# MayeulCassier/Matrix-Factorization-With-Comparison-Data

Measured on AMD Instinct MI355X. Metric: triplet-updates/sec, higher is better.
Workload: dtype f32

## Files before the change

matrix-factorization-with-comparison-data_amd/csrc/resident.hip:

```cpp
#include <cstring>
#include <mutex>
#include <utility>
#include <vector>

#include "resident_kernel.h"

#define MFCD_DECL(d)                                                                                                  \
    extern "C" int mfcd_resident_launch_d##d(const mfcd_detail::ResidentArgs *, int, int, void *) __attribute__((weak)); \
    extern "C" int mfcd_resident_occupancy_d##d(int, int, int, int) __attribute__((weak));
MFCD_DECL(2) MFCD_DECL(4) MFCD_DECL(8) MFCD_DECL(16) MFCD_DECL(32) MFCD_DECL(64) MFCD_DECL(128) MFCD_DECL(256)
#undef MFCD_DECL

namespace mfcd_detail {

int g_resident_math = 1;
Tuning g_tune;

typedef int (*ResidentLauncher)(const ResidentArgs *, int, int, void *);
typedef int (*ResidentOccupancy)(int, int, int, int);

static ResidentLauncher launcher_for(int d)
{
    switch (d) {
        case 2: return mfcd_resident_launch_d2;
        case 4: return mfcd_resident_launch_d4;
        case 8: return mfcd_resident_launch_d8;
        case 16: return mfcd_resident_launch_d16;
        case 32: return mfcd_resident_launch_d32;
        case 64: return mfcd_resident_launch_d64;
        case 128: return mfcd_resident_launch_d128;
        case 256: return mfcd_resident_launch_d256;
        default: return nullptr;
    }
}

static ResidentOccupancy occupancy_for(int d)
{
    switch (d) {
        case 2: return mfcd_resident_occupancy_d2;
        case 4: return mfcd_resident_occupancy_d4;
        case 8: return mfcd_resident_occupancy_d8;
        case 16: return mfcd_resident_occupancy_d16;
        case 32: return mfcd_resident_occupancy_d32;
        case 64: return mfcd_resident_occupancy_d64;
        case 128: return mfcd_resident_occupancy_d128;
        case 256: return mfcd_resident_occupancy_d256;
        default: return nullptr;
    }
}

int resident_lookahead(int64_t N, int B, int n, int m)
{
    int la = g_tune.lookahead >= 0 ? g_tune.lookahead : 4;
    if (B > 64) la = 0;
    if (N + 64 * 16 >= ((int64_t)1 << 31)) la = 0;
    if (g_tune.lookahead < 0 && (int64_t)(n + m) < (int64_t)96 * B) la = 0;
    return la > 16 ? 16 : (la < 0 ? 0 : la);
}

static int resident_blocks_per_cu(int d, int Q, int look, int fast, int bf16)
{
    static std::mutex mu;
    static std::vector<std::pair<long long, int>> cache;
    const long long key = ((((long long)d * 64 + Q) * 16 + look) * 2 + fast) * 2 + bf16;
    std::lock_guard<std::mutex> lock(mu);
    for (auto &e : cache)
        if (e.first == key) return e.second;
    int occ = 0;
    if (ResidentOccupancy fn = occupancy_for(d)) occ = fn(Q, look, fast, bf16);
    if (occ > 8) occ = 8;
    if (occ < 0) occ = 0;
    cache.emplace_back(key, occ);
    return occ;
}

static int resident_default_q(int n, int m, int d, int num_cus)
{
    if (d < 2 || d > 256 || (d & (d - 1)) != 0 || num_cus <= 0) return 0;
    const int64_t T = (int64_t)(n + m) * d;
    static const int kQ[5] = {1, 2, 4, 16, 32};
    for (int Q : kQ) {
        if ((64 * Q) % d != 0) continue;
        const int64_t nw = (T + 64 * (int64_t)Q - 1) / (64 * Q);
        if (nw <= (int64_t)num_cus * (Q <= 2 ? 16 : 8) && nw <= kResidentMaxWaves) return Q;
    }
    return 0;
}

ResidentEvents resident_events(int B, int n, int m, int d, int num_cus)
{
    ResidentEvents ev{0, 0, 0};
    const int Q = resident_default_q(n, m, d, num_cus);
    if (!Q || B > 64) return ev;
    ev.rows_per_wave = 64 * Q / d;
    ev.waves = (int)(((int64_t)(n + m) * d + 64 * (int64_t)Q - 1) / (64 * Q));
    const double h = 2.0 * 3.0 * B * ev.rows_per_wave / (double)(n + m);
    for (int ts = 8; ts >= 4; --ts)
        if (h * ((1 << ts) + kResidentEventLook) <= 20.0) {
            ev.tshift = ts;
            break;
        }
    return ev;
}

ResidentPlan plan_resident(int64_t N, int B, int n, int m, int d, int num_cus, bool bf16, int ev_tshift)
{
    ResidentPlan pl{};
    pl.ok = false;
    if (d < 2 || d > 256 || (d & (d - 1)) != 0 || num_cus <= 0 || !launcher_for(d)) return pl;
    const int64_t T = (int64_t)(n + m) * d;
    int look = resident_lookahead(N, B, n, m);
    const bool fast = g_resident_math != 0;
    if (ev_tshift < 0) ev_tshift = resident_events(B, n, m, d, num_cus).tshift;
    if (ev_tshift == 0) look = 0;
    static const int kQ[5] = {1, 2, 4, 16, 32};
    for (int qi = 0; qi < 5; ++qi) {
        const int Q = kQ[qi];
        if ((64 * Q) % d != 0) continue;
        const int64_t nw = (T + 64 * (int64_t)Q - 1) / (64 * Q);
        if (nw <= (int64_t)num_cus * (Q <= 2 ? 16 : 8) && nw <= kResidentMaxWaves) {
            const int occ = resident_blocks_per_cu(d, Q, look, fast, bf16);
            const int blocks = (int)((nw + 3) / 4);
            if (occ > 0 && (int64_t)blocks > (int64_t)occ * num_cus) continue;
            pl.ok = true;
            pl.Q = Q;
            pl.NW = (int)nw;
            pl.blocks = blocks;
            pl.lookahead = look;
            pl.fast_math = fast;
            pl.bf16 = bf16;
            pl.tshift = ev_tshift;
            return pl;
        }
    }
    return pl;
}

constexpr int kInlineStageUnits = 232;
struct InlineStage {
    uint4 v[kInlineStageUnits];
};

size_t train_inline_stage_bytes() { return (size_t)kInlineStageUnits * 16; }

template <bool INLINE>
__global__ __launch_bounds__(256) void train_prologue_kernel(InlineStage inl, const uint4 *__restrict__ stage_host,
                                                             uint4 *__restrict__ stage_dev, int stage_units,
                                                             const mfcd_sample *__restrict__ samples, int64_t N, int B,
                                                             int n, int m, int rows_per_wave, int tshift, int look,
                                                             int64_t nch_cap, mfcd_sample *__restrict__ xs,
                                                             unsigned *__restrict__ ev_cnt, uint4 *__restrict__ ev_ent)
{
    const int64_t t = (int64_t)blockIdx.x * blockDim.x + threadIdx.x;
    if (t < stage_units) {
        if constexpr (INLINE) {
            const uint4 *ka = (const uint4 *)__builtin_amdgcn_kernarg_segment_ptr();
            stage_dev[t] = ka[t];
        } else {
            stage_dev[t] = stage_host[t];
        }
    }
    if (!xs || t >= N) return;
    const RowMap rm = make_row_map(n, m);
    mfcd_sample s = samples[t];
    s.u = rm.vrow_u(s.u);
    s.i = rm.vrow_v(s.i);
    s.j = rm.vrow_v(s.j);
    xs[t] = s;
    if (look <= 0) return;
    const int k = (int)(t / B);
    const unsigned tl = (unsigned)(t - (int64_t)k * B);
    const int w[3] = {s.u / rows_per_wave, s.i / rows_per_wave, s.j / rows_per_wave};
    const unsigned lr[3] = {(unsigned)(s.u - w[0] * rows_per_wave), (unsigned)(s.i - w[1] * rows_per_wave),
                            (unsigned)(s.j - w[2] * rows_per_wave)};
    const int c = k >> tshift;
    const bool copy_back = c > 0 && (k & ((1 << tshift) - 1)) < look;
    uint4 e[3];
    size_t list[3];
    bool need[3];
#pragma unroll
    for (int r = 0; r < 3; ++r) {
        bool first = true;
#pragma unroll
        for (int r2 = 0; r2 < r; ++r2) first = first && w[r2] != w[r];
        need[r] = first;
        unsigned own = 0u, rows = 0u;
#pragma unroll
        for (int r2 = r; r2 < 3; ++r2)
            if (w[r2] == w[r]) {
                own |= 1u << r2;
                rows |= lr[r2] << (10 * r2);
            }
        e[r] = make_uint4(((unsigned)k << 9) | (tl << 3) | own, rows, __float_as_uint(s.z), 0u);
        list[r] = (size_t)w[r] * (size_t)nch_cap + (size_t)c;
    }
    unsigned slot[3] = {0u, 0u, 0u}, slot_back[3] = {0u, 0u, 0u};
#pragma unroll
    for (int r = 0; r < 3; ++r) {
        if (need[r]) slot[r] = atomicAdd(ev_cnt + list[r], 1u);
        if (need[r] && copy_back) slot_back[r] = atomicAdd(ev_cnt + list[r] - 1, 1u);
    }
#pragma unroll
    for (int r = 0; r < 3; ++r) {
        if (need[r] && slot[r] < (unsigned)kEventCap - 1u) ev_ent[list[r] * kEventCap + slot[r]] = e[r];
        if (need[r] && copy_back && slot_back[r] < (unsigned)kEventCap - 1u)
            ev_ent[(list[r] - 1) * kEventCap + slot_back[r]] = e[r];
    }
}

int launch_train_prologue(const void *stage_host, const void *stage_host_devview, void *stage_dev, size_t stage_bytes,
                          const mfcd_sample *samples, int64_t N, int B, int n, int m, int rows_per_wave, int tshift,
                          int look, int64_t nch_cap, mfcd_sample *xs, unsigned *ev_cnt, void *ev_ent, hipStream_t st)
{
    const int units = (int)((stage_bytes + 15) / 16);
    const int64_t items = xs ? (N > units ? N : units) : units;
    constexpr int kPT = 64;
    const dim3 grid((unsigned)((items + kPT - 1) / kPT));
    if (units <= kInlineStageUnits) {
        InlineStage inl;
        std::memcpy(inl.v, stage_host, (size_t)units * 16);
        hipLaunchKernelGGL(train_prologue_kernel<true>, grid, dim3(kPT), 0, st, inl, (const uint4 *)nullptr,
                           (uint4 *)stage_dev, units, samples, N, B, n, m, rows_per_wave, tshift, look, nch_cap, xs,
                           ev_cnt, (uint4 *)ev_ent);
    } else {
        static const InlineStage none{};
        hipLaunchKernelGGL(train_prologue_kernel<false>, grid, dim3(kPT), 0, st, none, (const uint4 *)stage_host_devview,
                           (uint4 *)stage_dev, units, samples, N, B, n, m, rows_per_wave, tshift, look, nch_cap, xs,
                           ev_cnt, (uint4 *)ev_ent);
    }
    MFCD_HIP_TRY(hipGetLastError());
    return 0;
}

int launch_resident_steps(const ResidentPlan &pl, const void *cold_dev, const mfcd_sample *xs, int64_t N, int B, int n,
                          int m, int d, const StepScalars *sc_dev, const AdamStatic &ac, unsigned long long *mailbox,
                          unsigned tag_base, void *loss_terms, unsigned long long *dbg, int K, hipStream_t st)
{
    ResidentArgs a;
    a.dbg = dbg;
    a.cold = (const ResidentCold *)cold_dev;
    a.samples = xs; a.sc = sc_dev; a.mailbox = mailbox; a.loss_terms = loss_terms;
    a.N = N; a.B = B; a.n = n; a.m = m; a.K = K; a.NW = pl.NW; a.ac = ac;
    a.lookahead = pl.lookahead;
    a.tag_base = tag_base;
    a.fast_math = pl.fast_math;
    a.bf16 = pl.bf16;
    ResidentLauncher fn = launcher_for(d);
    if (!fn) return MFCD_EINVAL;
    return fn(&a, pl.Q, pl.blocks, (void *)st);
}

}
```

matrix-factorization-with-comparison-data_amd/csrc/resident_kernel.h:

```cpp
#pragma once
#include "common.h"
#include "train_common.h"

namespace mfcd_detail {

typedef unsigned long long u64;

#define MFCD_LAMBDA_INLINE __attribute__((always_inline))

#ifdef MFCD_RES_STATS
#define RS_NOW() ((u64)__builtin_amdgcn_s_memtime())
#define RS_ADD(slot, val) rs_acc[slot] += (u64)(val)
#else
#define RS_NOW() ((u64)0)
#define RS_ADD(slot, val) ((void)0)
#endif

typedef const __attribute__((address_space(4))) float *ScalarTablePtr;
__device__ __forceinline__ StepScalars load_step_scalars(const StepScalars *table, int k)
{
    const ScalarTablePtr f = (ScalarTablePtr)(table + k);
    StepScalars s;
    s.neg_step_size = f[0];
    s.bc2_sqrt = f[1];
    s.inv_bc2_sqrt = f[2];
    s.pad = 0.0f;
    return s;
}


__device__ __forceinline__ u64 pack_granule(unsigned tag, float v)
{
    return ((u64)tag << 32) | (u64)__float_as_uint(v);
}

__device__ __forceinline__ u64 load_granule(const u64 *p)
{
    return __hip_atomic_load(p, __ATOMIC_RELAXED, __HIP_MEMORY_SCOPE_AGENT);
}

__device__ __forceinline__ void store_granule(u64 *p, unsigned tag, float v)
{
    __hip_atomic_store(p, pack_granule(tag, v), __ATOMIC_RELAXED, __HIP_MEMORY_SCOPE_AGENT);
}

struct RowMap {
    int n, m, c;
    __host__ __device__ int vrow_u(int u) const { return u < c ? 2 * u : 2 * c + (u - c); }
    __host__ __device__ int vrow_v(int i) const { return i < c ? 2 * i + 1 : 2 * c + (i - c); }
    __host__ __device__ int users_below(int x) const
    {
        if (x <= 2 * c) return (x + 1) >> 1;
        return n > c ? c + (x - 2 * c) : c;
    }
    __host__ __device__ int items_below(int x) const
    {
        if (x <= 2 * c) return x >> 1;
        return m > c ? c + (x - 2 * c) : c;
    }
    __host__ __device__ bool is_item(int vr) const { return vr < 2 * c ? (vr & 1) != 0 : m > n; }
    __host__ __device__ int table_row(int vr) const { return vr < 2 * c ? vr >> 1 : c + (vr - 2 * c); }
};
__host__ __device__ inline RowMap make_row_map(int n, int m)
{
    RowMap r;
    r.n = n; r.m = m; r.c = n < m ? n : m;
    return r;
}

constexpr int kEventCap = 64;
constexpr unsigned kEventNone = 0xFFFFFFF8u;
constexpr int kEventMaxLocalRows = 1024;

struct ResidentCold {
    float *U, *V, *mU, *vU, *mV, *vV;
    int *status;
    unsigned long long spin_limit;
    unsigned *ev_cnt;
    uint4 *ev_ent;
    long long nch_cap;
    long long tshift;
    float *loss_out;
    unsigned long long pad[3];
};
static_assert(sizeof(ResidentCold) == 128, "train.hip fills this block as sixteen 8-byte words (kColdBytes)");

struct ResidentArgs {
    const ResidentCold *cold;
    const mfcd_sample *samples;
    const StepScalars *sc;
    u64 *mailbox;
    void *loss_terms;
    u64 *dbg;
    unsigned tag_base;
    int64_t N;
    int B, n, m, K, NW;
    int lookahead;
    int fast_math;
    int bf16;
    AdamStatic ac;
};

__device__ __forceinline__ mfcd_sample load_record(const mfcd_sample *__restrict__ samples, int64_t pos0, int Bk,
                                                   int base, int lane)
{
    mfcd_sample s;
    s.u = s.i = s.j = -0x40000000;
    s.z = 0.0f;
    if (base + lane < Bk) s = samples[pos0 + base + lane];
    return s;
}

struct Masks {
    u64 mu, mi, mj;
};

template <int D, int Q, int LOOK, bool FAST, bool BF16 = false>
__global__ __launch_bounds__(256) __attribute__((amdgpu_waves_per_eu(Q >= 16 ? 2 : 1)))
void resident_train_kernel(ResidentArgs a)
{
    constexpr int S = D >= 64 ? D / 64 : 1;
    constexpr int RPR = D < 64 ? 64 / D : 1;
    constexpr int EW = 64 * Q;
    static_assert(EW % D == 0, "a wave's slice must hold whole rows");
    static_assert(EW / D <= kEventMaxLocalRows, "local row indices are 10-bit fields of an event entry");
    constexpr bool GRL = Q >= 16;
    extern __shared__ __attribute__((aligned(16))) float lds_dyn[];
    const int lane = threadIdx.x & 63;
    const int gw = blockIdx.x * (blockDim.x >> 6) + (threadIdx.x >> 6);
    if (gw >= a.NW) return;

    const int64_t T = (int64_t)(a.n + a.m) * D;
    const int64_t ebase = (int64_t)gw * EW;
    const int Rlo = (int)(ebase / D);
    const int64_t eend = (ebase + EW < T) ? ebase + EW : T;
    const int Rhi = (int)(eend / D);
    const int lcol = lane & (D - 1);
    auto elem_is_item = [&](int64_t e) MFCD_LAMBDA_INLINE { return make_row_map(a.n, a.m).is_item((int)(e / D)); };
    auto elem_offset = [&](int64_t e) MFCD_LAMBDA_INLINE { return (int64_t)make_row_map(a.n, a.m).table_row((int)(e / D)) * D + (e % D); };

#ifdef MFCD_RES_STATS
    u64 rs_acc[8] = {0, 0, 0, 0, 0, 0, 0, 0};
    const u64 rs_t0 = RS_NOW();
    [[maybe_unused]] const u64 rs_abs_t0 = __builtin_amdgcn_s_memrealtime();
    [[maybe_unused]] u64 rs_abs_l0 = 0, rs_abs_l1 = 0;
    [[maybe_unused]] u64 rs_hit[8] = {0, 0, 0, 0, 0, 0, 0, 0};
    [[maybe_unused]] u64 rs_mark = 0;
#endif
    float p[Q], m1[Q], m2[Q], gr[GRL ? 1 : Q];
    float *const lgr = lds_dyn + (threadIdx.x >> 6) * (GRL ? EW : 0);
    auto post = [](float x) MFCD_LAMBDA_INLINE {
        if constexpr (BF16) return (float)(mfcd_bf16)x;
        else return x;
    };
    {
        const ResidentCold c = *a.cold;
#pragma unroll
        for (int q = 0; q < Q; ++q) {
            const int64_t e = ebase + q * 64 + lane;
            p[q] = m1[q] = m2[q] = 0.0f;
            if constexpr (GRL) lgr[q * 64 + lane] = 0.0f;
            if (e < T) {
                const int64_t o = elem_offset(e);
                if (!elem_is_item(e)) { p[q] = BF16 ? (float)((const mfcd_bf16 *)c.U)[o] : c.U[o]; m1[q] = c.mU[o]; m2[q] = c.vU[o]; }
                else { p[q] = BF16 ? (float)((const mfcd_bf16 *)c.V)[o] : c.V[o]; m1[q] = c.mV[o]; m2[q] = c.vV[o]; }
            }
        }
    }

    auto batch_size = [&](int step) MFCD_LAMBDA_INLINE {
        const int64_t pos0 = (int64_t)step * a.B;
        return (int)((a.N - pos0) < a.B ? (a.N - pos0) : a.B);
    };
    auto scan = [&](const mfcd_sample &s, int Bk, int base) MFCD_LAMBDA_INLINE {
        const bool valid = base + lane < Bk;
        const int ru = s.u, ri = s.i, rj = s.j;
        Masks M;
        M.mu = __ballot(valid && ru >= Rlo && ru < Rhi);
        M.mi = __ballot(valid && ri >= Rlo && ri < Rhi);
        M.mj = __ballot(valid && rj >= Rlo && rj < Rhi);
        return M;
    };
    auto reg_of = [&](int lr) MFCD_LAMBDA_INLINE { return D >= 64 ? lr * S : lr / RPR; };

    auto give_up = [&](int step, int64_t pos, int what) MFCD_LAMBDA_INLINE {
        int *const status = a.cold->status;
        if (lane == 0) {
            if (__hip_atomic_exchange(status, 1, __ATOMIC_RELAXED, __HIP_MEMORY_SCOPE_AGENT) == 0 && a.dbg) {
                a.dbg[0] = (u64)gw; a.dbg[1] = (u64)step; a.dbg[2] = (u64)pos; a.dbg[3] = (u64)what;
            }
        }
    };
    auto poll_failed = [&](unsigned &spins, unsigned &limit) MFCD_LAMBDA_INLINE -> bool {
        if (spins == 0) limit = (unsigned)a.cold->spin_limit;
        ++spins;
        if (spins > limit || (spins & 255u) == 0) {
            if (spins > limit ||
                __hip_atomic_load(a.cold->status, __ATOMIC_RELAXED, __HIP_MEMORY_SCOPE_AGENT) != 0)
                return true;
        }
        return false;
    };

    auto store_row = [&](int lr, int64_t slot, unsigned tag) MFCD_LAMBDA_INLINE {
        u64 *dst = a.mailbox + slot * D;
        const int q0 = reg_of(lr);
#pragma unroll
        for (int q = 0; q < Q; ++q) {
            if (q >= q0 && q < q0 + S) {
                if constexpr (D >= 64) {
                    store_granule(dst + (q - q0) * 64 + lane, tag, p[q]);
                } else {
                    if (lane / D == lr % RPR) store_granule(dst + lcol, tag, p[q]);
                }
            }
        }
    };

    auto process_hit = [&](bool own0, bool own1, bool own2, int lr0, int lr1, int lr2, float zz, int64_t pos,
                           unsigned tag, float inv_batch, int step) MFCD_LAMBDA_INLINE -> bool {
        const bool own[3] = {own0, own1, own2};
        const int lrs[3] = {lr0, lr1, lr2};
        const u64 *slot = a.mailbox + pos * 3 * D;

        float row[3][S];
#pragma unroll
        for (int r = 0; r < 3; ++r) {
#pragma unroll
            for (int s2 = 0; s2 < S; ++s2) row[r][s2] = 0.0f;
            if (!own[r]) continue;
            const int q0 = reg_of(lrs[r]);
            if constexpr (D >= 64) {
#pragma unroll
                for (int q = 0; q < Q; ++q)
                    if (q >= q0 && q < q0 + S) row[r][(q * 64 % D) / 64] = p[q];
            } else {
                float sel = 0.0f;
#pragma unroll
                for (int q = 0; q < Q; ++q) sel = (q == q0) ? p[q] : sel;
                const float v = __shfl(sel, (lrs[r] % RPR) * D + lcol, MFCD_WAVE);
                row[r][0] = lane < D ? v : 0.0f;
            }
        }
        unsigned spins = 0, limit = 0;
        [[maybe_unused]] u64 rs_w0 = 0;
        RS_ADD(4, 1ull);
#ifdef MFCD_RES_STAMPS
        { const u64 t = RS_NOW(); rs_hit[0] += t - rs_mark; rs_mark = t; }
#endif
#if defined(MFCD_RES_STAGGER) && MFCD_RES_STAGGER > 0
        {
            u64 ga[3][S], gb[3][S];
            auto issue = [&](u64 (&g)[3][S]) MFCD_LAMBDA_INLINE {
#pragma unroll
                for (int r = 0; r < 3; ++r) {
                    if (own[r]) continue;
#pragma unroll
                    for (int s2 = 0; s2 < S; ++s2) {
                        const int c = lane + 64 * s2;
                        if (c < D) g[r][s2] = load_granule(slot + (int64_t)r * D + c);
                    }
                }
            };
            auto check = [&](const u64 (&g)[3][S]) MFCD_LAMBDA_INLINE -> bool {
                bool ok = true;
#pragma unroll
                for (int r = 0; r < 3; ++r) {
                    if (own[r]) continue;
#pragma unroll
                    for (int s2 = 0; s2 < S; ++s2) {
                        const int c = lane + 64 * s2;
                        if (c < D) {
                            ok = ok && ((unsigned)(g[r][s2] >> 32) == tag);
                            row[r][s2] = __uint_as_float((unsigned)g[r][s2]);
                        }
                    }
                }
                return __all(ok);
            };
            issue(ga);
            if (!check(ga)) {
#ifdef MFCD_RES_STATS
                rs_w0 = RS_NOW();
#endif
                issue(ga);
                __builtin_amdgcn_s_sleep(MFCD_RES_STAGGER);
                issue(gb);
                while (true) {
                    RS_ADD(5, 1);
                    if (poll_failed(spins, limit)) {
                        give_up(step, pos, (own0 ? 1 : 0) | (own1 ? 2 : 0) | (own2 ? 4 : 0));
                        return false;
                    }
                    if (check(ga)) break;
                    issue(ga);
                    if (check(gb)) break;
                    issue(gb);
                }
            }
        }
#else
        while (true) {
            bool ok = true;
#pragma unroll
            for (int r = 0; r < 3; ++r) {
                if (own[r]) continue;
#pragma unroll
                for (int s2 = 0; s2 < S; ++s2) {
                    const int c = lane + 64 * s2;
                    if (c < D) {
                        const u64 gq = load_granule(slot + (int64_t)r * D + c);
                        ok = ok && ((unsigned)(gq >> 32) == tag);
                        row[r][s2] = __uint_as_float((unsigned)gq);
                    }
                }
            }
            if (__all(ok)) break;
#ifdef MFCD_RES_STATS
            if (spins == 0) rs_w0 = RS_NOW();
            RS_ADD(5, 1);
#endif
            if (poll_failed(spins, limit)) {
                give_up(step, pos, (own0 ? 1 : 0) | (own1 ? 2 : 0) | (own2 ? 4 : 0));
                return false;
            }
        }
#endif
#ifdef MFCD_RES_STATS
        if (spins) RS_ADD(2, RS_NOW() - rs_w0);
        else RS_ADD(4, 1ull << 40);
#endif
#ifdef MFCD_RES_STAMPS
        { const u64 t = RS_NOW(); rs_hit[1] += t - rs_mark; if (!spins) { rs_hit[6] += t - rs_mark; rs_hit[7] += 1; } rs_mark = t; }
#endif

        float acc = 0.0f;
#pragma unroll
        for (int s2 = 0; s2 < S; ++s2) acc += row[0][s2] * (row[1][s2] - row[2][s2]);
        float pr, g;
        if constexpr (FAST) {
            const float x = wave_sum64(acc);
            const float e = __builtin_amdgcn_exp2f(x * -1.44269504088896340736f);
            const float dn = 1.0f + e;
            pr = div_newton(1.0f, dn, __builtin_amdgcn_rcpf(dn));
            pr = (e == __builtin_inff()) ? 0.0f : pr;
            const float den = fmaxf((1.0f - pr) * pr, 1e-12f);
            const float num = inv_batch * (pr - zz);
            g = div_newton(num, den, __builtin_amdgcn_rcpf(den)) * (1.0f - pr) * pr;
        } else {
            pr = sigmoid_f32(wave_sum64(acc));
            g = bce_sigmoid_backward_f32(pr, zz, inv_batch);
        }
        if (own[0] && lane == 0) {
            if constexpr (LOOK > 0) store_granule((u64 *)a.loss_terms + pos, tag, pr);
            else ((float *)a.loss_terms)[pos] = pr;
        }

        float du[S], dv[S];
#pragma unroll
        for (int s2 = 0; s2 < S; ++s2) {
            du[s2] = g * (row[1][s2] - row[2][s2]);
            dv[s2] = g * row[0][s2];
        }
        if constexpr (D < 64) {
            du[0] = __shfl(du[0], lcol, MFCD_WAVE);
            dv[0] = __shfl(dv[0], lcol, MFCD_WAVE);
        }
        if constexpr (GRL) {
#pragma unroll
            for (int r = 0; r < 3; ++r) {
                if (!own[r]) continue;
                const int q0 = reg_of(lrs[r]);
                if constexpr (D >= 64) {
#pragma unroll
                    for (int s2 = 0; s2 < S; ++s2)
                        lgr[(q0 + s2) * 64 + lane] += r == 0 ? du[s2] : (r == 1 ? dv[s2] : -dv[s2]);
                } else {
                    if (lane / D == lrs[r] % RPR) lgr[q0 * 64 + lane] += r == 0 ? du[0] : (r == 1 ? dv[0] : -dv[0]);
                }
            }
        } else {
#pragma unroll
            for (int q = 0; q < Q; ++q) {
                const int rowq = (q * 64 + lane) / D;
                const int sq = D >= 64 ? (q * 64 % D) / 64 : 0;
                if (own[0] && rowq == lrs[0]) gr[q] += du[sq];
                if (own[1] && rowq == lrs[1]) gr[q] += dv[sq];
                if (own[2] && rowq == lrs[2]) gr[q] += -dv[sq];
            }
        }
#ifdef MFCD_RES_STAMPS
        { const u64 t = RS_NOW(); rs_hit[2] += t - rs_mark; rs_mark = t; }
#endif
        return true;
    };

    auto step_update = [&](bool hit, const StepScalars &sc) MFCD_LAMBDA_INLINE {
        if constexpr (GRL) {
            if (hit) {
#pragma unroll
                for (int q = 0; q < Q; ++q) {
                    const float g = lgr[q * 64 + lane];
                    lgr[q * 64 + lane] = 0.0f;
                    adam_update_t<FAST>(p[q], m1[q], m2[q], g, a.ac, sc);
                    p[q] = post(p[q]);
                }
            } else {
#pragma unroll
                for (int q = 0; q < Q; ++q) {
                    adam_update_t<FAST>(p[q], m1[q], m2[q], 0.0f, a.ac, sc);
                    p[q] = post(p[q]);
                }
            }
        } else {
            adam_update_q<FAST, Q, false>(p, m1, m2, gr, a.ac, sc);
            if constexpr (BF16) {
#pragma unroll
                for (int q = 0; q < Q; ++q) p[q] = post(p[q]);
            }
        }
    };

    auto generic_loop = [&]() MFCD_LAMBDA_INLINE -> bool {
        auto publish = [&](int step) MFCD_LAMBDA_INLINE {
            const int64_t pos0 = (int64_t)step * a.B;
            const int Bk = batch_size(step);
            for (int base = 0; base < Bk; base += MFCD_WAVE) {
                const mfcd_sample s = load_record(a.samples, pos0, Bk, base, lane);
                const Masks M = scan(s, Bk, base);
                u64 mask = M.mu | M.mi | M.mj;
                while (mask) {
                    const int tl = __ffsll((long long)mask) - 1;
                    mask &= mask - 1;
                    const int64_t slot0 = (pos0 + base + tl) * 3;
                    if ((M.mu >> tl) & 1ull) store_row(__shfl(s.u, tl, MFCD_WAVE) - Rlo, slot0 + 0, a.tag_base + (unsigned)step + 1u);
                    if ((M.mi >> tl) & 1ull) store_row(__shfl(s.i, tl, MFCD_WAVE) - Rlo, slot0 + 1, a.tag_base + (unsigned)step + 1u);
                    if ((M.mj >> tl) & 1ull) store_row(__shfl(s.j, tl, MFCD_WAVE) - Rlo, slot0 + 2, a.tag_base + (unsigned)step + 1u);
                }
            }
        };
        publish(0);
        for (int k = 0; k < a.K; ++k) {
            const int64_t pos0 = (int64_t)k * a.B;
            const int Bk = batch_size(k);
            const float inv_batch = 1.0f / (float)Bk;
            const StepScalars sc = load_step_scalars(a.sc, k);
            if constexpr (!GRL) {
#pragma unroll
                for (int q = 0; q < Q; ++q) gr[q] = 0.0f;
            }
            bool any_hit = false;
            for (int base = 0; base < Bk; base += MFCD_WAVE) {
                const mfcd_sample s = load_record(a.samples, pos0, Bk, base, lane);
                const Masks M = scan(s, Bk, base);
                u64 mask = M.mu | M.mi | M.mj;
                any_hit = any_hit || mask != 0ull;
                while (mask) {
                    const int tl = __ffsll((long long)mask) - 1;
                    mask &= mask - 1;
                    const int hu = __shfl(s.u, tl, MFCD_WAVE) - Rlo, hi = __shfl(s.i, tl, MFCD_WAVE) - Rlo,
                              hj = __shfl(s.j, tl, MFCD_WAVE) - Rlo;
                    const float hz = __shfl(s.z, tl, MFCD_WAVE);
                    const bool ok = process_hit((bool)((M.mu >> tl) & 1ull), (bool)((M.mi >> tl) & 1ull),
                                                (bool)((M.mj >> tl) & 1ull), hu, hi, hj, hz, pos0 + base + tl,
                                                a.tag_base + (unsigned)k + 1u, inv_batch, k);
                    if (__builtin_amdgcn_readfirstlane((int)!ok)) return false;
                }
            }
            step_update(any_hit, sc);
            if (k + 1 < a.K) publish(k + 1);
        }
        return true;
    };

    bool alive = true;

    if constexpr (LOOK > 0) {
        const int W = __builtin_amdgcn_readfirstlane(a.lookahead);
        const int N32 = (int)a.N;
        const int gws = __builtin_amdgcn_readfirstlane(gw);
        const int tshift = (int)a.cold->tshift;
        const int NCH = ((a.K - 1) >> tshift) + 1;

        bool fits = true;
        {
            const unsigned *cnt = a.cold->ev_cnt + (size_t)gws * (size_t)a.cold->nch_cap;
            for (int c = lane; c < NCH; c += MFCD_WAVE) fits = fits && cnt[c] < (unsigned)kEventCap;
            fits = __all(fits);
        }
        if (!__builtin_amdgcn_readfirstlane((int)fits)) {
            alive = generic_loop();
        } else {
            unsigned ekey = kEventNone, erow = 0u;
            int estep = 0x7FFFFF;
            float ez = 0.0f;
            int chunk_end = 0;

            auto load_chunk = [&](int c) MFCD_LAMBDA_INLINE {
                const ResidentCold *cz = a.cold;
                const size_t li = (size_t)gws * (size_t)cz->nch_cap + (size_t)c;
                const uint4 e = cz->ev_ent[li * kEventCap + lane];
                const unsigned n_raw = cz->ev_cnt[li];
                const unsigned n = (unsigned)__builtin_amdgcn_readfirstlane((int)n_raw);
                const unsigned key = (unsigned)lane < n ? e.x : kEventNone;
                unsigned rank = 0u;
                for (unsigned l = 0; l < n; ++l) {
                    const unsigned kl = (unsigned)__builtin_amdgcn_readlane((int)key, (int)l);
                    rank += kl < key ? 1u : 0u;
                }
                const int dest = (int)((unsigned)lane < n ? rank : (unsigned)lane) << 2;
                ekey = (unsigned)__builtin_amdgcn_ds_permute(dest, (int)key);
                erow = (unsigned)__builtin_amdgcn_ds_permute(dest, (int)e.y);
                ez = __builtin_bit_cast(float, __builtin_amdgcn_ds_permute(dest, (int)e.z));
                estep = (int)(ekey >> 9);
                const int ce = (c + 1) << tshift;
                chunk_end = ce < a.K ? ce : a.K;
            };
            auto step_at = [&](int i) MFCD_LAMBDA_INLINE -> int { return __builtin_amdgcn_readlane(estep, i); };
            auto lanes_in = [](int lo, int hi) MFCD_LAMBDA_INLINE -> u64 { return ((1ull << hi) - 1ull) & ~((1ull << lo) - 1ull); };
            auto rowmask = [&](int lr) MFCD_LAMBDA_INLINE -> u64 {
                const bool t = ((ekey & 1u) && (int)(erow & 1023u) == lr) ||
                               ((ekey & 2u) && (int)((erow >> 10) & 1023u) == lr) ||
                               ((ekey & 4u) && (int)((erow >> 20) & 1023u) == lr);
                return __ballot(t);
            };

            auto publish_entry = [&](int idx, int jbase, int conf_lo, int conf_hi, int touch_lo, int touch_hi,
                                     bool need_touch) MFCD_LAMBDA_INLINE {
                const unsigned key_l = (unsigned)__builtin_amdgcn_readlane((int)ekey, idx);
                const unsigned row_l = (unsigned)__builtin_amdgcn_readlane((int)erow, idx);
                const int ke = (int)(key_l >> 9);
                const int tl = (int)((key_l >> 3) & 63u);
#pragma unroll 1
                for (int r = 0; r < 3; ++r) {
                    if (!((key_l >> r) & 1u)) continue;
                    const int lr = (int)((row_l >> (10 * r)) & 1023u);
                    if (conf_lo < conf_hi || need_touch) {
                        const u64 rm = rowmask(lr);
                        if (rm & lanes_in(conf_lo, conf_hi)) continue;
                        if (need_touch && !(rm & lanes_in(touch_lo, touch_hi))) continue;
                    }
                    const int q0 = reg_of(lr);
                    float pp[S], mm1[S], mm2[S];
#pragma unroll
                    for (int s2 = 0; s2 < S; ++s2) pp[s2] = mm1[s2] = mm2[s2] = 0.0f;
#pragma unroll
                    for (int q = 0; q < Q; ++q) {
                        if (q >= q0 && q < q0 + S) {
                            const int s2 = D >= 64 ? (q * 64 % D) / 64 : 0;
                            pp[s2] = p[q];
                            mm1[s2] = m1[q];
                            mm2[s2] = m2[q];
                        }
                    }
                    StepScalars scb = load_step_scalars(a.sc, jbase + 1);
#pragma unroll 1
                    for (int st = jbase + 1; st < ke; ++st) {
                        const StepScalars scn = load_step_scalars(a.sc, st + 1);
#pragma unroll
                        for (int s2 = 0; s2 < S; ++s2) {
                            adam_update_t<FAST>(pp[s2], mm1[s2], mm2[s2], 0.0f, a.ac, scb);
                            pp[s2] = post(pp[s2]);
                        }
                        scb = scn;
                    }
                    u64 *dst = a.mailbox + (((int64_t)ke * a.B + tl) * 3 + r) * D;
                    const unsigned tag = a.tag_base + (unsigned)ke + 1u;
                    if constexpr (D >= 64) {
#pragma unroll
                        for (int s2 = 0; s2 < S; ++s2) store_granule(dst + s2 * 64 + lane, tag, pp[s2]);
                    } else {
                        if (lane / D == lr % RPR) store_granule(dst + lcol, tag, pp[0]);
                    }
                    RS_ADD(7, 1);
                }
            };
            auto publish_fresh = [&](int jbase, int lo, int hi, int touch_lo, int touch_hi) MFCD_LAMBDA_INLINE {
                if (lo >= hi) return;
                [[maybe_unused]] const u64 rs_p0 = RS_NOW();
                int g0 = lo, gstep = step_at(lo);
                for (int idx = lo; idx < hi; ++idx) {
                    const int st = step_at(idx);
                    if (st != gstep) { g0 = idx; gstep = st; }
                    publish_entry(idx, jbase, lo, g0, touch_lo, touch_hi, jbase >= 0);
                }
                RS_ADD(3, RS_NOW() - rs_p0);
            };
            load_chunk(0);
            int hc = 0, pc = __builtin_popcountll(__ballot(estep < W));
            publish_fresh(-1, 0, pc, 0, 0);
            int nh = step_at(0), np = step_at(pc);
            auto next_event = [&]() MFCD_LAMBDA_INLINE -> int {
                const int cp = np - W;
                const int e = nh < cp ? nh : cp;
                return e < chunk_end ? e : chunk_end;
            };
            int next_evt = next_event();

            ScalarTablePtr scp = (ScalarTablePtr)a.sc;
            auto load_scalars_at = [&](ScalarTablePtr f) MFCD_LAMBDA_INLINE {
                StepScalars x;
                x.neg_step_size = f[0];
                x.bc2_sqrt = f[1];
                x.inv_bc2_sqrt = f[2];
                x.pad = 0.0f;
                return x;
            };
            StepScalars sc_cur = load_scalars_at(scp);
            int chunk = 0;
#ifdef MFCD_RES_STATS
            const u64 rs_l0 = RS_NOW();
            rs_acc[6] = rs_l0 - rs_t0;
            rs_abs_l0 = __builtin_amdgcn_s_memrealtime();
#endif
            int k = 0;
            while (true) {
                const int kq = next_evt < a.K ? next_evt : a.K;
                while (k < kq) {
                    scp += 4;
                    const StepScalars sc_next = load_scalars_at(scp);
                    if constexpr (GRL) {
                        step_update(false, sc_cur);
                    } else {
#pragma unroll
                        for (int q = 0; q < Q; ++q) {
                            adam_update_t<FAST>(p[q], m1[q], m2[q], 0.0f, a.ac, sc_cur);
                            p[q] = post(p[q]);
                        }
                    }
                    sc_cur = sc_next;
                    ++k;
                }
                if (k >= a.K) break;
                scp += 4;
                const StepScalars sc_next = load_scalars_at(scp);
                if constexpr (!GRL) {
#pragma unroll
                    for (int q = 0; q < Q; ++q) gr[q] = 0.0f;
                }
                bool hit = false;
                int h0 = 0;
                {
                    __builtin_amdgcn_s_setprio(3);
                    [[maybe_unused]] const u64 rs_e0 = RS_NOW();
#ifdef MFCD_RES_STAMPS
                    rs_mark = rs_e0;
#endif
                    RS_ADD(7, 1ull << 32);
                    if (k == chunk_end) {
                        load_chunk(++chunk);
                        hc = 0;
                        nh = step_at(0);
                        pc = __builtin_popcountll(__ballot(estep < k + W));
                        np = step_at(pc);
                    }
                    if (np == k + W) {
                        [[maybe_unused]] const u64 rs_p0 = RS_NOW();
                        const int g0 = pc;
                        do {
                            publish_entry(pc, k - 1, hc, g0, 0, 0, false);
                            ++pc;
                            np = step_at(pc);
                        } while (np == k + W);
                        RS_ADD(3, RS_NOW() - rs_p0);
                    }
                    h0 = hc;
                    if (nh == k) {
                        hit = true;
                        const int bk = (N32 - k * a.B) < a.B ? (N32 - k * a.B) : a.B;
                        const float inv_batch = 1.0f / (float)bk;
                        const unsigned tag = a.tag_base + (unsigned)k + 1u;
                        do {
                            const unsigned key_l = (unsigned)__builtin_amdgcn_readlane((int)ekey, hc);
                            const unsigned row_l = (unsigned)__builtin_amdgcn_readlane((int)erow, hc);
                            const float z_l = __builtin_bit_cast(float, __builtin_amdgcn_readlane(__builtin_bit_cast(int, ez), hc));
                            const bool ok = process_hit((bool)(key_l & 1u), (bool)(key_l & 2u), (bool)(key_l & 4u),
                                                        (int)(row_l & 1023u), (int)((row_l >> 10) & 1023u),
                                                        (int)((row_l >> 20) & 1023u), z_l,
                                                        (int64_t)k * a.B + (int)((key_l >> 3) & 63u), tag, inv_batch, k);
                            if (__builtin_amdgcn_readfirstlane((int)!ok)) { alive = false; break; }
                            ++hc;
                            nh = step_at(hc);
                        } while (nh == k);
                        if (!alive) break;
                    }
                    next_evt = next_event();
                    if (!hit) __builtin_amdgcn_s_setprio(0);
                    RS_ADD(1, RS_NOW() - rs_e0);
                }
                step_update(hit, sc_cur);
#ifdef MFCD_RES_STAMPS
                if (hit) { const u64 t = RS_NOW(); rs_hit[3] += t - rs_mark; rs_mark = t; }
#endif
                if (__builtin_expect(hit, 0)) {
                    publish_fresh(k, hc, pc, h0, hc);
                    __builtin_amdgcn_s_setprio(0);
#ifdef MFCD_RES_STAMPS
                    { const u64 t = RS_NOW(); rs_hit[4] += t - rs_mark; rs_hit[5] += 1; }
#endif
                }
                sc_cur = sc_next;
                ++k;
            }
            __builtin_amdgcn_s_setprio(0);
#ifdef MFCD_RES_STATS
            rs_abs_l1 = __builtin_amdgcn_s_memrealtime();
            rs_acc[0] = RS_NOW() - rs_l0;
            rs_acc[6] |= (u64)__builtin_amdgcn_s_getreg((31 << 11) | 4) << 32;
            rs_acc[5] |= (u64)__builtin_amdgcn_s_getreg((31 << 11) | 20) << 32;
            if (lane == 0 && a.dbg)
                for (int x = 0; x < 8; ++x) a.dbg[8 + (int64_t)gw * 8 + x] = rs_acc[x];
#endif
        }

        {
            float *const loss_out = a.cold->loss_out;
            if (loss_out != nullptr) {
                for (int k = gws; k < a.K && alive; k += a.NW) {
                    const int64_t off = (int64_t)k * a.B;
                    const int b = (int)((a.N - off) < a.B ? (a.N - off) : a.B);
                    const unsigned tag = a.tag_base + (unsigned)k + 1u;
                    const float zz = lane < b ? a.samples[off + lane].z : 0.0f;
                    unsigned spins = 0, limit = 0;
                    float pr = 0.0f;
                    while (true) {
                        bool ok = true;
                        if (lane < b) {
                            const u64 gq = load_granule((const u64 *)a.loss_terms + off + lane);
                            ok = (unsigned)(gq >> 32) == tag;
                            pr = __uint_as_float((unsigned)gq);
                        }
                        if (__all(ok)) break;
                        __builtin_amdgcn_s_sleep(8);
                        if (poll_failed(spins, limit)) {
                            give_up(k, off, 8);
                            alive = false;
                            break;
                        }
                    }
                    if (!alive) break;
                    float acc = lane < b ? bce_term_f32(pr, zz) : 0.0f;
                    acc = wave_sum64(acc);
                    if (lane == 0) loss_out[k] = acc / (float)b;
                }
            }
        }
        {
            unsigned *const cnt = a.cold->ev_cnt + (size_t)gws * (size_t)a.cold->nch_cap;
            for (int c = lane; c < NCH; c += MFCD_WAVE) cnt[c] = 0u;
        }
    } else {
        alive = generic_loop();
    }

    const ResidentCold c = *a.cold;
#pragma unroll
    for (int q = 0; q < Q; ++q) {
        const int64_t e = ebase + q * 64 + lane;
        if (e < T) {
            const int64_t o = elem_offset(e);
            if (!elem_is_item(e)) {
                if constexpr (BF16) ((mfcd_bf16 *)c.U)[o] = (mfcd_bf16)p[q];
                else c.U[o] = p[q];
                c.mU[o] = m1[q]; c.vU[o] = m2[q];
            } else {
                if constexpr (BF16) ((mfcd_bf16 *)c.V)[o] = (mfcd_bf16)p[q];
                else c.V[o] = p[q];
                c.mV[o] = m1[q]; c.vV[o] = m2[q];
            }
        }
    }
#ifdef MFCD_RES_STAMPS
    if (lane == 0 && a.dbg) {
        u64 *const o = a.dbg + 8 + (int64_t)gw * 8;
        o[1] = rs_abs_t0; o[2] = rs_abs_l0; o[3] = rs_abs_l1; o[7] = __builtin_amdgcn_s_memrealtime();
        for (int x = 0; x < 8; ++x) o[4096 * 8 + x] = rs_hit[x];
    }
#endif
}

}
```

Measured before the change: 92.89 million.

## Adapt wave priority to mailbox waiting and prefetch first event chunk

Each wave now tracks whether any mailbox poll had to spin. If a hit finished without spinning while more events are still pending, the wave keeps an elevated scheduling priority (2) in place of dropping to 0, so waves that hold up peers get more issue slots. The first event chunk's counts and entries are loaded during the prologue and reused for the capacity check, which also finds the last busy chunk. The per-step inverse batch size is precomputed on the host and passed as kernel arguments. The priority heuristic can starve other waves and may reduce throughput.

Measured after the change: 90.18 million. 0.971x the previous value.

```diff
diff --git a/matrix-factorization-with-comparison-data_amd/csrc/resident.hip b/matrix-factorization-with-comparison-data_amd/csrc/resident.hip
--- a/matrix-factorization-with-comparison-data_amd/csrc/resident.hip
+++ b/matrix-factorization-with-comparison-data_amd/csrc/resident.hip
@@ -245,6 +245,9 @@
     a.tag_base = tag_base;
     a.fast_math = pl.fast_math;
     a.bf16 = pl.bf16;
+    const int64_t last = N - (int64_t)(K - 1) * B;
+    a.inv_batch = 1.0f / (float)B;
+    a.inv_batch_last = 1.0f / (float)(last < B ? last : B);
     ResidentLauncher fn = launcher_for(d);
     if (!fn) return MFCD_EINVAL;
     return fn(&a, pl.Q, pl.blocks, (void *)st);
diff --git a/matrix-factorization-with-comparison-data_amd/csrc/resident_kernel.h b/matrix-factorization-with-comparison-data_amd/csrc/resident_kernel.h
--- a/matrix-factorization-with-comparison-data_amd/csrc/resident_kernel.h
+++ b/matrix-factorization-with-comparison-data_amd/csrc/resident_kernel.h
@@ -98,6 +98,8 @@
     int lookahead;
     int fast_math;
     int bf16;
+    float inv_batch;
+    float inv_batch_last;
     AdamStatic ac;
 };
 
@@ -153,8 +155,17 @@
         if constexpr (BF16) return (float)(mfcd_bf16)x;
         else return x;
     };
+    [[maybe_unused]] unsigned cnt_head = 0u;
+    [[maybe_unused]] const uint4 *ent_head = nullptr;
+    [[maybe_unused]] int tshift0 = 0;
     {
         const ResidentCold c = *a.cold;
+        if constexpr (LOOK > 0) {
+            tshift0 = (int)c.tshift;
+            const size_t l0 = (size_t)gw * (size_t)c.nch_cap;
+            if (lane <= ((a.K - 1) >> tshift0)) cnt_head = c.ev_cnt[l0 + (size_t)lane];
+            ent_head = c.ev_ent + l0 * kEventCap + lane;
+        }
 #pragma unroll
         for (int q = 0; q < Q; ++q) {
             const int64_t e = ebase + q * 64 + lane;
@@ -218,7 +229,7 @@
     };
 
     auto process_hit = [&](bool own0, bool own1, bool own2, int lr0, int lr1, int lr2, float zz, int64_t pos,
-                           unsigned tag, float inv_batch, int step) MFCD_LAMBDA_INLINE -> bool {
+                           unsigned tag, float inv_batch, int step, unsigned &spun) MFCD_LAMBDA_INLINE -> bool {
         const bool own[3] = {own0, own1, own2};
         const int lrs[3] = {lr0, lr1, lr2};
         const u64 *slot = a.mailbox + pos * 3 * D;
@@ -326,6 +337,7 @@
             }
         }
 #endif
+        spun |= spins;
 #ifdef MFCD_RES_STATS
         if (spins) RS_ADD(2, RS_NOW() - rs_w0);
         else RS_ADD(4, 1ull << 40);
@@ -461,9 +473,10 @@
                     const int hu = __shfl(s.u, tl, MFCD_WAVE) - Rlo, hi = __shfl(s.i, tl, MFCD_WAVE) - Rlo,
                               hj = __shfl(s.j, tl, MFCD_WAVE) - Rlo;
                     const float hz = __shfl(s.z, tl, MFCD_WAVE);
+                    unsigned spun = 0u;
                     const bool ok = process_hit((bool)((M.mu >> tl) & 1ull), (bool)((M.mi >> tl) & 1ull),
                                                 (bool)((M.mj >> tl) & 1ull), hu, hi, hj, hz, pos0 + base + tl,
-                                                a.tag_base + (unsigned)k + 1u, inv_batch, k);
+                                                a.tag_base + (unsigned)k + 1u, inv_batch, k, spun);
                     if (__builtin_amdgcn_readfirstlane((int)!ok)) return false;
                 }
             }
@@ -477,17 +490,26 @@
 
     if constexpr (LOOK > 0) {
         const int W = __builtin_amdgcn_readfirstlane(a.lookahead);
-        const int N32 = (int)a.N;
         const int gws = __builtin_amdgcn_readfirstlane(gw);
-        const int tshift = (int)a.cold->tshift;
+        const int tshift = __builtin_amdgcn_readfirstlane(tshift0);
         const int NCH = ((a.K - 1) >> tshift) + 1;
 
-        bool fits = true;
+        bool fits = cnt_head < (unsigned)kEventCap;
+        int last_busy = -1;
         {
+            const u64 busy = __ballot(cnt_head != 0u);
+            if (busy) last_busy = 63 - __builtin_clzll(busy);
+        }
+        if (NCH > MFCD_WAVE) {
             const unsigned *cnt = a.cold->ev_cnt + (size_t)gws * (size_t)a.cold->nch_cap;
-            for (int c = lane; c < NCH; c += MFCD_WAVE) fits = fits && cnt[c] < (unsigned)kEventCap;
-            fits = __all(fits);
-        }
+            for (int c0 = MFCD_WAVE; c0 < NCH; c0 += MFCD_WAVE) {
+                const unsigned nc = c0 + lane < NCH ? cnt[c0 + lane] : 0u;
+                fits = fits && nc < (unsigned)kEventCap;
+                const u64 busy = __ballot(nc != 0u);
+                if (busy) last_busy = c0 + 63 - __builtin_clzll(busy);
+            }
+        }
+        fits = __all(fits);
         if (!__builtin_amdgcn_readfirstlane((int)fits)) {
             alive = generic_loop();
         } else {
@@ -496,12 +518,7 @@
             float ez = 0.0f;
             int chunk_end = 0;
 
-            auto load_chunk = [&](int c) MFCD_LAMBDA_INLINE {
-                const ResidentCold *cz = a.cold;
-                const size_t li = (size_t)gws * (size_t)cz->nch_cap + (size_t)c;
-                const uint4 e = cz->ev_ent[li * kEventCap + lane];
-                const unsigned n_raw = cz->ev_cnt[li];
-                const unsigned n = (unsigned)__builtin_amdgcn_readfirstlane((int)n_raw);
+            auto sort_chunk = [&](int c, const uint4 &e, unsigned n) MFCD_LAMBDA_INLINE {
                 const unsigned key = (unsigned)lane < n ? e.x : kEventNone;
                 unsigned rank = 0u;
                 for (unsigned l = 0; l < n; ++l) {
@@ -515,6 +532,13 @@
                 estep = (int)(ekey >> 9);
                 const int ce = (c + 1) << tshift;
                 chunk_end = ce < a.K ? ce : a.K;
+            };
+            auto load_chunk = [&](int c) MFCD_LAMBDA_INLINE {
+                const ResidentCold *cz = a.cold;
+                const size_t li = (size_t)gws * (size_t)cz->nch_cap + (size_t)c;
+                const uint4 e = cz->ev_ent[li * kEventCap + lane];
+                const unsigned n_raw = cz->ev_cnt[li];
+                sort_chunk(c, e, (unsigned)__builtin_amdgcn_readfirstlane((int)n_raw));
             };
             auto step_at = [&](int i) MFCD_LAMBDA_INLINE -> int { return __builtin_amdgcn_readlane(estep, i); };
             auto lanes_in = [](int lo, int hi) MFCD_LAMBDA_INLINE -> u64 { return ((1ull << hi) - 1ull) & ~((1ull << lo) - 1ull); };
@@ -586,7 +610,7 @@
                 }
                 RS_ADD(3, RS_NOW() - rs_p0);
             };
-            load_chunk(0);
+            sort_chunk(0, *ent_head, (unsigned)__builtin_amdgcn_readlane((int)cnt_head, 0));
             int hc = 0, pc = __builtin_popcountll(__ballot(estep < W));
             publish_fresh(-1, 0, pc, 0, 0);
             int nh = step_at(0), np = step_at(pc);
@@ -608,6 +632,11 @@
             };
             StepScalars sc_cur = load_scalars_at(scp);
             int chunk = 0;
+            bool behind = false;
+            auto quiet_prio = [&]() MFCD_LAMBDA_INLINE {
+                if (behind) __builtin_amdgcn_s_setprio(2);
+                else __builtin_amdgcn_s_setprio(0);
+            };
 #ifdef MFCD_RES_STATS
             const u64 rs_l0 = RS_NOW();
             rs_acc[6] = rs_l0 - rs_t0;
@@ -640,6 +669,7 @@
                 }
                 bool hit = false;
                 int h0 = 0;
+                unsigned spun = 0u;
                 {
                     __builtin_amdgcn_s_setprio(3);
                     [[maybe_unused]] const u64 rs_e0 = RS_NOW();
@@ -667,8 +697,7 @@
                     h0 = hc;
                     if (nh == k) {
                         hit = true;
-                        const int bk = (N32 - k * a.B) < a.B ? (N32 - k * a.B) : a.B;
-                        const float inv_batch = 1.0f / (float)bk;
+                        const float inv_batch = k + 1 < a.K ? a.inv_batch : a.inv_batch_last;
                         const unsigned tag = a.tag_base + (unsigned)k + 1u;
                         do {
                             const unsigned key_l = (unsigned)__builtin_amdgcn_readlane((int)ekey, hc);
@@ -677,7 +706,7 @@
                             const bool ok = process_hit((bool)(key_l & 1u), (bool)(key_l & 2u), (bool)(key_l & 4u),
                                                         (int)(row_l & 1023u), (int)((row_l >> 10) & 1023u),
                                                         (int)((row_l >> 20) & 1023u), z_l,
-                                                        (int64_t)k * a.B + (int)((key_l >> 3) & 63u), tag, inv_batch, k);
+                                                        (int64_t)k * a.B + (int)((key_l >> 3) & 63u), tag, inv_batch, k, spun);
                             if (__builtin_amdgcn_readfirstlane((int)!ok)) { alive = false; break; }
                             ++hc;
                             nh = step_at(hc);
@@ -685,7 +714,7 @@
                         if (!alive) break;
                     }
                     next_evt = next_event();
-                    if (!hit) __builtin_amdgcn_s_setprio(0);
+                    if (!hit) quiet_prio();
                     RS_ADD(1, RS_NOW() - rs_e0);
                 }
                 step_update(hit, sc_cur);
@@ -694,7 +723,8 @@
 #endif
                 if (__builtin_expect(hit, 0)) {
                     publish_fresh(k, hc, pc, h0, hc);
-                    __builtin_amdgcn_s_setprio(0);
+                    behind = (bool)__builtin_amdgcn_readfirstlane((int)(spun == 0u && (nh != 0x7FFFFF || last_busy > chunk)));
+                    quiet_prio();
 #ifdef MFCD_RES_STAMPS
                     { const u64 t = RS_NOW(); rs_hit[4] += t - rs_mark; rs_hit[5] += 1; }
 #endif
```
